# JaapWijnen/metal-raytracing

Measured on AMD Instinct MI355X. Metric: Mrays/sec (primary+shadow) and ms/frame, DragonScene 1920x1080 spp=1, higher is better.
Workload: dtype f32

## Files before the change

metal-raytracing_amd/csrc/api.cpp:

```cpp
#include "api_types.h"
#include "abi_check.h"
#include "../../include/mrt_debug.h"
#include <algorithm>
#include <cstring>
#include <cstdio>
#include <memory>
#include <new>

namespace mrt {
static thread_local std::string g_err;
void set_error(const std::string &msg) { g_err = msg; }
int hip_fail(hipError_t e, const char *what, const char *file, int line) {
    char buf[512];
    snprintf(buf, sizeof buf, "HIP error %d (%s) in %s at %s:%d", (int)e, hipGetErrorString(e), what, file, line);
    g_err = buf;
    return e == hipErrorOutOfMemory ? MRT_ERR_OUT_OF_MEMORY : MRT_ERR_HIP;
}
}

static int bind_device(MRTContext ctx) { MRT_HIP(hipSetDevice(ctx->device)); return MRT_OK; }

static int sync_host_meshes(MRTScene scene) {
    bool pending = false;
    int rc = mrt::download_stale_meshes(scene->meshes, scene->dev, &pending);
// ... 723 lines not shown
    else { mrt::set_error("mrt_renderer_get_option: unknown key " + k); return MRT_ERR_INVALID_ARGUMENT; }
    return MRT_OK;
    MRT_CATCH
}
int mrt_debug_renderer_set_option(MRTRenderer r, const char *key, double value) {
    MRT_TRY
    REQUIRE(r && key, "mrt_debug_renderer_set_option: bad argument");
    std::string k(key);
    if (k == "persistent") { REQUIRE(value == 0 || value == 1 || value == 2, "persistent must be 0 (never), 1 (always) or 2 (by launch size)"); r->r.persistent = (int)value; }
    else if (k == "xcd_counters") { REQUIRE(value == 0 || value == 1, "xcd_counters must be 0 or 1"); r->r.xcd_counters = (int)value; }
    else if (k == "tile_groups") { REQUIRE(value >= 0 && value <= mrt::MAX_TILE_GROUPS && value == (int)value, "tile_groups must be 0 (by the draw), 1 (never) or 2..4"); r->r.tile_groups = (int)value; }
    else if (k == "shade_pack") { REQUIRE(value == 0 || value == 1, "shade_pack must be 0 or 1"); r->r.shade_pack = (int)value; }
    else if (k == "hit_lds") { REQUIRE(value == 0 || value == 1, "hit_lds must be 0 or 1"); r->r.hit_lds = (int)value; }
    else if (k == "persist_chunk") { REQUIRE(value >= 64 && value <= 65536 && ((int)value % 64) == 0, "persist_chunk must be a multiple of 64 in [64, 65536]"); r->r.persist_chunk = (int)value; }
    else if (k == "wave_slots") { REQUIRE(value >= 1 && value <= (1 << 20), "wave_slots must be in [1, 2^20]"); r->r.wave_slots = (int)value; r->r.wave_slots_user = true; }
    else if (k == "stream_stride") { REQUIRE(value >= 0 && value <= 2, "stream_stride must be 0 (contiguous ranges), 1 (round-robin batches) or 2 (round-robin for a shard's launches)"); r->r.stream_stride = (int)value; }
    else if (k == "halton_table") r->r.halton_table = value != 0;
    else if (k == "equal_passes") r->r.equal_passes = value != 0;
    else if (k == "frame_bundle") { REQUIRE(value == 0 || value == 1, "frame_bundle must be 0 (off) or 1 (the sub-frames of a slot side by side in a wave)"); r->r.frame_bundle = (int)value; }
    else if (k == "stream_even") { REQUIRE(value >= 0 && value <= 1600, "stream_even must be in [0,1600] (percent of the wave slots; 0 = off)"); r->r.stream_even = (int)value; }
    else if (k == "primary_hint") r->r.primary_hint = value != 0;
    else if (k == "throughput_chain") r->r.throughput_chain = value != 0;
    else if (k == "shadow_planes") r->r.shadow_planes = value != 0 ? 1 : 0;
    else if (k == "tail_accumulate") r->r.tail_accumulate = value != 0;
    else if (k == "fuse_primary") { REQUIRE(value == 0 || value == 1 || value == 2, "fuse_primary must be 0, 1 (not for one frame alone) or 2 (always)"); r->r.fuse_primary = (int)value; }
    else if (k == "wide_bounce") r->r.wide_bounce = value != 0;
    else if (k == "tl_pair_cap") { REQUIRE(value >= 0 && value <= 4294967295.0, "tl_pair_cap out of range"); r->r.tl_pair_cap = (int)std::min(value, 2147483647.0); }
    else if (k == "tl_pairs") { REQUIRE(value == 0 || value == 1 || value == 2, "tl_pairs must be 0 (two-level scenes walked in one loop), 1 (TLAS pass + BLAS pass over (ray, instance) pairs) or 2 (the same, the TLAS pass always as a walk of the 8-wide TLAS)"); r->r.tl_pairs = (int)value; }
    else if (k == "primary_wide") { REQUIRE(value == 0 || value == 1 || value == 2, "primary_wide must be 0 (rope walk inside shade(0)), 1 (own launch of the 8-wide stream kernel) or 2 (8-wide walk inside shade(0))"); r->r.primary_wide = (int)value; }
    else return mrt_renderer_set_option(r, key, value);
    return MRT_OK;
    MRT_CATCH
}
int mrt_debug_renderer_get_option(MRTRenderer r, const char *key, double *value) {
    MRT_TRY
    REQUIRE(r && key && value, "mrt_debug_renderer_get_option: bad argument");
    std::string k(key);
    if (k == "persistent") *value = r->r.persistent;
    else if (k == "persist_chunk") *value = r->r.persist_chunk;
    else if (k == "hit_lds") *value = r->r.hit_lds;
    else if (k == "shade_pack") *value = r->r.shade_pack;
    else if (k == "tile_groups") *value = r->r.tile_groups;
    else if (k == "groups_used") *value = r->r.groups_used;
    else if (k == "xcd_counters") *value = r->r.xcd_counters;
    else if (k == "wave_slots") *value = r->r.wave_slots;
    else if (k == "stream_stride") *value = r->r.stream_stride;
    else if (k == "halton_table") *value = r->r.halton_table;
    else if (k == "frame_bundle") *value = r->r.frame_bundle;
    else if (k == "stream_even") *value = r->r.stream_even;
    else if (k == "primary_hint") *value = r->r.primary_hint ? 1 : 0;
    else if (k == "throughput_chain") *value = r->r.throughput_chain ? 1 : 0;
    else if (k == "shadow_planes") *value = r->r.shadow_planes;
    else if (k == "tail_accumulate") *value = r->r.tail_accumulate ? 1 : 0;
    else if (k == "fuse_primary") *value = r->r.fuse_primary;
    else if (k == "wide_bounce") *value = r->r.wide_bounce ? 1 : 0;
    else if (k == "tl_pairs") *value = r->r.tl_pairs;
    else if (k == "tl_pair_cap") *value = r->r.tl_pair_cap;
    else if (k == "primary_wide") *value = r->r.primary_wide;
    else return mrt_renderer_get_option(r, key, value);
    return MRT_OK;
    MRT_CATCH
}
int mrt_renderer_set_shard(MRTRenderer r, int32_t rank, int32_t world) {
    MRT_TRY
    RENDERER_PROLOGUE("mrt_renderer_set_shard")
    return r->r.set_shard(rank, world);
    MRT_CATCH
}
int mrt_renderer_set_frame_index(MRTRenderer r, uint32_t fi) { REQUIRE(r, "mrt_renderer_set_frame_index: NULL"); r->r.frame_index = fi; return MRT_OK; }
int mrt_renderer_frame_index(MRTRenderer r, uint32_t *fi) { REQUIRE(r && fi, "mrt_renderer_frame_index: bad argument"); *fi = r->r.frame_index; return MRT_OK; }
int mrt_renderer_render(MRTRenderer r, int32_t n_frames) {
    MRT_TRY
    RENDERER_PROLOGUE("mrt_renderer_render")
    REQUIRE(n_frames >= 0, "mrt_renderer_render: n_frames < 0");
    if (!r->scene->committed) { mrt::set_error("mrt_renderer_render: scene was modified and not re-committed"); return MRT_ERR_STATE; }
    if (n_frames == 0) return MRT_OK;
// ... 265 lines not shown
```

metal-raytracing_amd/csrc/renderer.h:

```cpp
#pragma once
#include "scene_device.h"
#include "host_geometry.h"
#include <algorithm>
#include <array>
#include <deque>
#include <vector>

namespace mrt {

struct EvPair { hipEvent_t a = nullptr, b = nullptr; int kind = 0; };

struct FrameLane {
    hipStream_t stream = nullptr;
    hipEvent_t accumulated = nullptr;
    DevBuf<float4> sample;
    DevBuf<float4> rayA[2], rayB[2], thr[2], hits, srayA, srayB, scon;
    DevBuf<unsigned long long> bounce_counts;
    DevBuf<float4> f_con[2];
    DevBuf<uint8_t> f_lit;
    DevBuf<uint4> pairs;
};
constexpr int MAX_FRAMES_IN_FLIGHT = 16;
constexpr int MAX_TILE_GROUPS = 4;
struct TileGroup { int rank = 0, world = 1, tiles_local = 0; uint32_t capacity = 0; uint64_t owned = 0; const uint32_t *seeds = nullptr; };
// ... 34 lines not shown
    uint32_t mega_waves = 0;
};
struct SlotCache { size_t lds_bytes = ~(size_t)0; int per_cu = 0; };
struct DrawCtx;

struct Renderer {
    hipStream_t stream = nullptr;
    const DeviceScene *scene = nullptr;
    int width = 0, height = 0, max_bounces = 3;
    uint32_t seed = 1;
    MRTCamera camera{};
    uint32_t frame_index = 0;
    uint32_t sample_offset = 0;
    int cur = 0;
    int shard_rank = 0, shard_world = 1;
    int tiles_local = 0;
    uint32_t capacity = 0;
    uint64_t owned_pixels = 0;
    uint64_t frames_rendered = 0;

    DevBuf<uint32_t> seeds;
    DevBuf<float> halton_tab;
    uint32_t halton_w0 = 0;
    int halton_table = 1;
    int ensure_halton_table(uint32_t sample_index, uint32_t frames);
    DevBuf<uint32_t> hint;
    bool primary_hint = true;
    bool throughput_chain = true;
    DevBuf<float4> accum[2];
    FrameLane lanes[MAX_FRAMES_IN_FLIGHT];
    int frames_in_flight = 3;
    int frame_batch = 0;
    int batch_wanted() const;
    int tile_groups = 0;
    int groups_used = 1;
    TileGroup tgroups[MAX_TILE_GROUPS];
    DevBuf<uint32_t> seeds_g[MAX_TILE_GROUPS]; int tgroups_for = 0, tgroups_batch = 0;
    int ensure_tile_groups(int G);
    int lanes_used = 0;
    int lanes_ready = 0;
    int alloc_batch = 0;
    bool megakernel = false;
    bool materials = false;
    int primary_wide = 2;
    int persistent = 2;
    int xcd_counters = 1;
    int hit_lds = 1;
    int shade_pack = 1;
    int persist_chunk = 256;
    int wave_slots = 7168;
    bool wave_slots_user = false;
    mutable SlotCache mega_cache, persist_cache, persist_x_cache;
    mutable int cu_count = 0;
    int alloc_planes(FrameLane &L);
    bool tail_accumulate = true;
    int fuse_primary = 1;
    int shadow_planes = 1;
    int equal_passes = 1;
    int frame_bundle = 1;
    int stream_stride = 2;
    int stream_even = 200;
    int tl_pair_cap = 0;
    int tl_pairs = 1;
    bool wide_bounce = true;
    hipEvent_t ev_fork = nullptr;
    DevBuf<unsigned long long> totals;

    bool guides = false;
    bool guides_valid = false;
    bool guides_keep = false;
    DevBuf<float4> guide_nd, guide_albedo; DevBuf<int4> guide_ids;
    hipStream_t guide_stream = nullptr;
    hipEvent_t guide_fork = nullptr, guide_done = nullptr;
    DevBuf<float4> dn_scratch[2], denoised; bool denoised_valid = false;
    int set_guides(bool on);
    int ensure_guides();
    int clear_guides();
    int read_guide(int which, void *out, size_t nbytes);
// ... 14 lines not shown
    hipEvent_t ev_begin = nullptr, ev_end = nullptr;
    std::array<EvPair, 512> ev_ext;
    int ext_used = 0;
    bool pending_timing = false;
    float ms_last = 0, ms_extend_last = 0; uint32_t extend_launches_last = 0;
    MRTKernelTimes kernel_times{};

    Renderer() = default;
    Renderer(const Renderer &) = delete;
    ~Renderer();
    int init(hipStream_t st, const DeviceScene *sc, int w, int h, uint32_t seed, int max_bounces);
    int resize(int w, int h);
    int alloc_queues();
    int alloc_lane(FrameLane &L);
    void release_lane(FrameLane &L);
    size_t lane_bytes() const;
    int set_shard(int rank, int world);
    int render(int n_frames);
    DrawPlan plan_draw(int n_frames) const;
    int plan_pass(const DrawPlan &dp, const SceneView &sv, const TileGroup &TG, int B, PassPlan &pp) const;
    PullGrid pull_grid(size_t slots, size_t slots_of_chip, size_t min_chunk, bool long_call) const;
    int draw_nothing(int n_frames);
    int rebuild_for_batch();
    int ensure_lanes(int want);
    void begin_draw(DrawCtx &d) const;
    int prepare_lane(FrameLane &L, const TileGroup &TG, const PassPlan &pp);
    int enqueue_pass(DrawCtx &d, FrameLane &L, const TileGroup &TG, const PassPlan &pp, int pass, int g);
    int enqueue_megakernel_pass(DrawCtx &d, FrameLane &L, const TileGroup &TG, const PassPlan &pp);
    void enqueue_primary(DrawCtx &d, FrameLane &L, const TileGroup &TG, const PassPlan &pp);
    void enqueue_shade(DrawCtx &d, FrameLane &L, const TileGroup &TG, const PassPlan &pp, int b);
    void enqueue_trace(DrawCtx &d, FrameLane &L, const TileGroup &TG, const PassPlan &pp, int b);
    int enqueue_accumulate(DrawCtx &d, FrameLane &L, const TileGroup &TG, const PassPlan &pp, int pass, int g);
    int enqueue_guides(DrawCtx &d);
    EvPair *timed(int kind);
    int wait();
    int read_accum(float *rgba, size_t nbytes);
    int copy_accum_to_device(void *dptr, size_t nbytes);
    int write_accum_from_device(const void *dptr, size_t nbytes);
    int read_tonemapped(uint8_t *rgba, size_t nbytes);
    int pack_owned_tiles(void *dptr, size_t nbytes);
    int unpack_tiles(const void *dptr, size_t nbytes, int rank, int world);
    int stats(MRTRenderStats *out);
    int reset_stats();
};

uint32_t shard_tiles(int width, int height, int rank, int world);
int unpack_tiles_into(float4 *image, int width, int height, const void *compact, size_t nbytes, int rank, int world, hipStream_t st);
// ... 15 lines not shown
```

metal-raytracing_amd/csrc/renderer.hip:

```cpp
#include <hip/hip_ext.h>
#include "renderer.h"
#include "device_math.h"
#include "traverse.h"
#include "traverse_wide.h"
#include "traverse_instanced.h"
#include "shade.h"
#include "two_level_passes.h"
#include <cstdlib>
#include <cstring>
#include <algorithm>

namespace mrt {
namespace {

__global__ void k_halton_table(float *__restrict__ tab, uint32_t w0, uint32_t n) {
    const uint32_t j = blockIdx.x * blockDim.x + threadIdx.x;
    if (j < n) tab[MRT_HALTON_INTERLEAVED ? (size_t)j * HALTON_TAB_DIMS + blockIdx.y : (size_t)blockIdx.y * n + j] = halton_dev((int)(w0 + j), (int)blockIdx.y + 1);
}

__global__ void k_seed(uint32_t *__restrict__ seeds, uint32_t n, uint32_t seed) {
    uint32_t i = blockIdx.x * blockDim.x + threadIdx.x;
    if (i < n) seeds[(size_t)blockIdx.y * n + i] = seed_hash_dev(seed, i) + blockIdx.y;
}

// ... 583 lines not shown

static inline uint32_t cdiv(size_t a, size_t b) { return (uint32_t)((a + b - 1) / b); }

template <class... KArgs, class... Args>
static inline void launch_timed(EvPair *ev, void (*kernel)(KArgs...), dim3 grid, dim3 block, size_t shmem, hipStream_t st, Args... args) {
    if (ev) hipExtLaunchKernelGGL(kernel, grid, block, (uint32_t)shmem, st, ev->a, ev->b, 0, static_cast<KArgs>(args)...);
    else hipLaunchKernelGGL(kernel, grid, block, shmem, st, static_cast<KArgs>(args)...);
}

}

#ifdef MRT_WAVE_TIMES
int read_wave_times(unsigned long long *out) { return hipMemcpyFromSymbol(out, HIP_SYMBOL(g_wave_times), sizeof(g_wave_times)) == hipSuccess ? MRT_OK : MRT_ERR_HIP; }
int read_wave_iters(uint32_t *out) { return hipMemcpyFromSymbol(out, HIP_SYMBOL(g_wave_iters), sizeof(g_wave_iters)) == hipSuccess ? MRT_OK : MRT_ERR_HIP; }
int read_drain_probe(unsigned long long *out18, int reset) {
    if (hipMemcpyFromSymbol(out18, HIP_SYMBOL(g_drain_probe), sizeof(g_drain_probe)) != hipSuccess) return MRT_ERR_HIP;
    if (reset) { static const unsigned long long z[18] = {0}; if (hipMemcpyToSymbol(HIP_SYMBOL(g_drain_probe), z, sizeof z) != hipSuccess) return MRT_ERR_HIP; }
    return MRT_OK;
}
#endif

int Renderer::ensure_halton_table(uint32_t sample_index, uint32_t frames) {
    const uint64_t first_pass = std::min<uint64_t>(frames, MAX_FRAME_BATCH);
    const bool fits = halton_tab.p != nullptr && sample_index >= halton_w0 && (uint64_t)sample_index + first_pass + (1u << 20) <= (uint64_t)halton_w0 + HALTON_TAB_SPAN;
    if (fits) return MRT_OK;
    if (!halton_tab.p) MRT_HIP(halton_tab.alloc((size_t)HALTON_TAB_DIMS * HALTON_TAB_SPAN));
    halton_w0 = sample_index;
    hipLaunchKernelGGL(k_halton_table, dim3(cdiv(HALTON_TAB_SPAN, 256), HALTON_TAB_DIMS), dim3(256), 0, stream, halton_tab.p, halton_w0, HALTON_TAB_SPAN);
    MRT_HIP(hipGetLastError());
    return MRT_OK;
}

int Renderer::init(hipStream_t st, const DeviceScene *sc, int w, int h, uint32_t seed_, int max_bounces_) {
    stream = st; scene = sc; seed = seed_; max_bounces = max_bounces_;
    MRT_HIP(hipEventCreate(&ev_begin)); MRT_HIP(hipEventCreate(&ev_end));
    MRT_HIP(hipEventCreateWithFlags(&ev_fork, hipEventDisableTiming));
    for (auto &e : ev_ext) { MRT_HIP(hipEventCreate(&e.a)); MRT_HIP(hipEventCreate(&e.b)); }
    for (auto &L : lanes) {
        MRT_HIP(hipStreamCreateWithFlags(&L.stream, hipStreamNonBlocking));
        MRT_HIP(hipEventCreateWithFlags(&L.accumulated, hipEventDisableTiming));
        MRT_HIP(L.bounce_counts.alloc(WORK_COUNTERS + 32 * WORK_COUNTERS_PER_BOUNCE));
        MRT_HIP(hipMemsetAsync(L.bounce_counts.p, 0, L.bounce_counts.bytes(), stream));
    }
    MRT_HIP(totals.alloc(4));
    MRT_HIP(hipMemsetAsync(totals.p, 0, totals.bytes(), stream));
    return resize(w, h);
}

Renderer::~Renderer() {
    if (ev_begin) (void)hipEventDestroy(ev_begin);
    if (ev_end) (void)hipEventDestroy(ev_end);
    if (ev_fork) (void)hipEventDestroy(ev_fork);
    for (auto &e : ev_ext) { if (e.a) (void)hipEventDestroy(e.a); if (e.b) (void)hipEventDestroy(e.b); }
    for (auto &pd : passes_pending) (void)hipEventDestroy(pd.ev);
    for (auto e : pass_events_free) (void)hipEventDestroy(e);
    if (guide_stream) { (void)hipStreamSynchronize(guide_stream); (void)hipStreamDestroy(guide_stream); }
    if (guide_done) (void)hipEventDestroy(guide_done);
    if (guide_fork) (void)hipEventDestroy(guide_fork);
    for (auto &L : lanes) {
        if (L.stream) { (void)hipStreamSynchronize(L.stream); (void)hipStreamDestroy(L.stream); }
        if (L.accumulated) (void)hipEventDestroy(L.accumulated);
    }
}

int Renderer::batch_wanted() const {
    if (frame_batch > 0) return std::min(frame_batch, MAX_FRAME_BATCH);
    const size_t owned = std::max<size_t>(1, (size_t)std::max(width, 1) * (size_t)std::max(height, 1) / (size_t)std::max(shard_world, 1));
    const size_t ref = (size_t)DEFAULT_FRAME_BATCH * 1920 * 1080;
// ... 101 lines not shown
    for (int k = 0; k < 2; k++) { MRT_HIP(L.rayA[k].alloc(qcap)); MRT_HIP(L.rayB[k].alloc(qcap)); if (need_thr) MRT_HIP(L.thr[k].alloc(qcap)); }
    MRT_HIP(L.hits.alloc(qcap)); MRT_HIP(L.srayA.alloc(qcap)); MRT_HIP(L.srayB.alloc(qcap));
    if (need_thr || !shadow_planes) MRT_HIP(L.scon.alloc(qcap));
    MRT_HIP(L.sample.alloc((size_t)std::max<uint32_t>(capacity, 1u) * (size_t)std::max(1, alloc_batch)));
    MRT_HIP(hipMemsetAsync(L.sample.p, 0, L.sample.bytes(), stream));
    if (shadow_planes && !need_thr) { if (int rc = alloc_planes(L)) return rc; }
    return MRT_OK;
}

int Renderer::ensure_tile_groups(int G) {
    const int Bq = std::max(1, alloc_batch);
    if (tgroups_for == G && tgroups_batch == Bq) return MRT_OK;
    const int tiles_x = (width + 7) / 8, tiles_y = (height + 7) / 8, tiles = tiles_x * tiles_y;
    for (int g = 0; g < G; g++) {
        TileGroup &T = tgroups[g];
        T.rank = g * shard_world + shard_rank; T.world = G * shard_world;
        T.tiles_local = std::max(0, (tiles - T.rank + T.world - 1) / T.world);
        T.capacity = (uint32_t)T.tiles_local * 64u;
        T.owned = 0;
        for (int lt = 0; lt < T.tiles_local; lt++) {
            const int tile = lt * T.world + T.rank, ty = tile / tiles_x, tx = tile % tiles_x;
            T.owned += (uint64_t)std::min(8, width - tx * 8) * (uint64_t)std::min(8, height - ty * 8);
        }
        MRT_HIP(seeds_g[g].alloc((size_t)std::max<uint32_t>(T.capacity, 1u) * Bq));
        FrameParams sp{}; sp.width = width; sp.height = height; sp.shard_rank = T.rank; sp.shard_world = T.world; sp.tiles_x = tiles_x; sp.tiles_local = T.tiles_local; sp.capacity = T.capacity;
        if (T.capacity) hipLaunchKernelGGL(k_seed_slots, dim3(cdiv(T.capacity, 256), Bq), dim3(256), 0, stream, seeds_g[g].p, sp, seed);
        T.seeds = seeds_g[g].p;
    }
    tgroups_for = G; tgroups_batch = Bq;
    return MRT_OK;
}

int Renderer::set_shard(int rank, int world) {
    if (world < 1 || rank < 0 || rank >= world) { set_error("invalid shard"); return MRT_ERR_INVALID_ARGUMENT; }
    shard_rank = rank; shard_world = world;
    MRT_HIP(hipStreamSynchronize(stream));
    MRT_HIP(hipMemsetAsync(accum[0].p, 0, accum[0].bytes(), stream));
    MRT_HIP(hipMemsetAsync(accum[1].p, 0, accum[1].bytes(), stream));
    frame_index = 0; cur = 0;
    if (int rc = clear_guides()) return rc;
    return alloc_queues();
}

int Renderer::clear_guides() {
    guides_valid = false; denoised_valid = false;
    if (guide_nd.p) {
        MRT_HIP(hipMemsetAsync(guide_nd.p, 0, guide_nd.bytes(), stream)); MRT_HIP(hipMemsetAsync(guide_albedo.p, 0, guide_albedo.bytes(), stream));
        MRT_HIP(hipMemsetAsync(guide_ids.p, 0, guide_ids.bytes(), stream));
    }
    return MRT_OK;
}
int Renderer::set_guides(bool on) {
// ... 67 lines not shown
    int rc = wait(); if (rc) return rc;
    MRT_HIP(hipMemcpy(rgba, tmp.p, nbytes, hipMemcpyDeviceToHost));
    return MRT_OK;
}

#ifdef MRT_DIAGNOSTICS
static inline int ablate_mask() { static const int mask = getenv("MRT_ABLATE") ? atoi(getenv("MRT_ABLATE")) : 0; return mask; }
#else
static constexpr int ablate_mask() { return 0; }
#endif
static inline uint32_t tag_bounce(uint32_t arg, int b) {
#ifdef MRT_WAVE_TIMES
    return arg | ((uint32_t)b << 24);
#else
    (void)b; return arg;
#endif
}

struct DrawCtx {
    SceneView sv;
    DrawPlan dp;
    FrameParams fp;
    FrameParams gp;
    hipEvent_t last_acc, last_acc_g[MAX_TILE_GROUPS];
    AccGroup tail;
};

template <class K>
static int wave_slots_for(K kernel, size_t lds_bytes, SlotCache &cache, int &cu_count) {
    if (cu_count == 0) { int dev = 0; hipDeviceProp_t prop; MRT_HIP(hipGetDevice(&dev)); MRT_HIP(hipGetDeviceProperties(&prop, dev)); cu_count = prop.multiProcessorCount; }
    if (cache.lds_bytes != lds_bytes) { MRT_HIP(hipOccupancyMaxActiveBlocksPerMultiprocessor(&cache.per_cu, kernel, 64, lds_bytes)); cache.lds_bytes = lds_bytes; }
    return MRT_OK;
}

EvPair *Renderer::timed(int kind) { if (ext_used >= (int)ev_ext.size()) return nullptr; ev_ext[ext_used].kind = kind; return &ev_ext[ext_used++]; }

DrawPlan Renderer::plan_draw(int n_frames) const {
    DrawPlan dp;
    dp.n_frames = n_frames; dp.mega = megakernel; dp.equal = equal_passes != 0; dp.tail = tail_accumulate;
    const int batch_cap = alloc_batch > DEFAULT_FRAME_BATCH ? std::min(alloc_batch, std::max(DEFAULT_FRAME_BATCH, (n_frames + 2) / 3)) : alloc_batch;
    dp.batch_max = megakernel ? 1 : batch_cap;
    dp.n_passes = (n_frames + dp.batch_max - 1) / dp.batch_max;
    dp.lanes = dp.lanes_plain = std::max(1, std::min(frames_in_flight, MAX_FRAMES_IN_FLIGHT));
    if (!megakernel && tile_groups != 1 && tiles_local >= 64) {
        const int in_flight = std::max(1, std::min(dp.lanes, dp.n_passes));
        const int by_draw = tile_groups >= 2 ? tile_groups : dp.batch_max > 1 ? 1 : in_flight == 1 ? 3 : in_flight <= 3 ? 2 : 1;
        dp.G = std::max(1, std::min(by_draw, std::min(MAX_FRAMES_IN_FLIGHT / in_flight, tiles_local / 32)));
        if (dp.G > 1) dp.lanes = in_flight * dp.G;
    }
    return dp;
}

void DrawPlan::settle(int lanes_ready) {
    if (G > 1 && lanes_ready < lanes) { G = 1; lanes = lanes_plain; }
    lanes = std::min(lanes, lanes_ready);
    Fp = G > 1 ? lanes / G : lanes;
    tail_from = (tail && G == 1) ? n_passes - std::min(lanes, n_passes) : n_passes;
    long_call = n_passes >= 2 * lanes;
}

PullGrid Renderer::pull_grid(size_t slots, size_t slots_of_chip, size_t min_chunk, bool long_call) const {
    PullGrid pg;
    pg.chunk = (uint32_t)std::min<size_t>((size_t)persist_chunk, std::max<size_t>(min_chunk, slots / (slots_of_chip * 4) / 64 * 64));
    pg.grid_slots = (!wave_slots_user && long_call) ? std::max<size_t>(1, slots_of_chip / 2) : slots_of_chip;
    pg.waves = (uint32_t)std::max<size_t>(1, std::min<size_t>(cdiv(slots, pg.chunk), pg.grid_slots));
    return pg;
// ... 74 lines not shown
    return MRT_OK;
}

int Renderer::rebuild_for_batch() {
    MRT_HIP(hipStreamSynchronize(stream));
    const uint32_t keep_frame = frame_index; const int keep_cur = cur; const uint64_t keep_rendered = frames_rendered;
    DevBuf<float4> keep; MRT_HIP(keep.alloc(accum[cur].n));
    MRT_HIP(hipMemcpyAsync(keep.p, accum[cur].p, accum[cur].bytes(), hipMemcpyDeviceToDevice, stream));
    const MRTCamera keep_cam = camera;
    unsigned long long keep_totals[3] = {0, 0, 0};
    MRT_HIP(hipMemcpy(keep_totals, totals.p, sizeof keep_totals, hipMemcpyDeviceToHost));
    const bool keep_denoised = denoised_valid;
    guides_keep = true;
    int rc = resize(width, height);
    guides_keep = false; denoised_valid = keep_denoised;
    if (rc) return rc;
    MRT_HIP(hipMemcpyAsync(totals.p, keep_totals, sizeof keep_totals, hipMemcpyHostToDevice, stream));
    MRT_HIP(hipMemcpyAsync(accum[keep_cur].p, keep.p, keep.bytes(), hipMemcpyDeviceToDevice, stream));
    MRT_HIP(hipStreamSynchronize(stream));
    frame_index = keep_frame; cur = keep_cur; frames_rendered = keep_rendered; frames_completed_known = keep_rendered; camera = keep_cam;
    return MRT_OK;
}

int Renderer::ensure_lanes(int want) {
    for (; lanes_ready < want; lanes_ready++) {
        const size_t need = lane_bytes() + (lanes_ready == 0 && !halton_tab.p ? (size_t)HALTON_TAB_DIMS * HALTON_TAB_SPAN * sizeof(float) : 0);
        size_t free_b = 0, total_b = 0;
        const bool fits = hipMemGetInfo(&free_b, &total_b) != hipSuccess || free_b > need + (size_t(1) << 30);
        int rc = fits ? alloc_lane(lanes[lanes_ready]) : MRT_ERR_OUT_OF_MEMORY;
        if (rc == MRT_ERR_OUT_OF_MEMORY && lanes_ready >= 1) { (void)hipGetLastError(); release_lane(lanes[lanes_ready]); break; }
        if (rc == MRT_ERR_OUT_OF_MEMORY) { set_error("not enough device memory for one pass in flight: " + std::to_string(need >> 20) + " MiB of ray queues needed (" + std::to_string(width) + "x" + std::to_string(height) + ", frame_batch " + std::to_string(alloc_batch) + "); lower frame_batch"); return rc; }
        if (rc) return rc;
    }
    return MRT_OK;
}

void Renderer::begin_draw(DrawCtx &d) const {
    FrameParams &fp = d.fp;
    fp = FrameParams{};
    fp.width = width; fp.height = height; fp.lightCount = light_count_limit > 0 ? std::min(light_count_limit, d.sv.light_count) : d.sv.light_count;
    fp.cam_pos = make_float4(camera.position.x, camera.position.y, camera.position.z, 0);
    fp.cam_right = make_float4(camera.right.x, camera.right.y, camera.right.z, 0);
    fp.cam_up = make_float4(camera.up.x, camera.up.y, camera.up.z, 0);
    fp.cam_fwd = make_float4(camera.forward.x, camera.forward.y, camera.forward.z, 0);
    fp.shard_rank = shard_rank; fp.shard_world = shard_world;
    fp.tiles_x = (width + 7) / 8; fp.tiles_local = tiles_local; fp.max_bounces = max_bounces;
    d.gp = fp;
    d.gp.frameIndex = frame_index; d.gp.sampleIndex = frame_index + sample_offset; d.gp.npix = (uint32_t)((size_t)width * height); d.gp.capacity = capacity; d.gp.batch = 1;
    fp.npix = (uint32_t)((size_t)width * height); fp.capacity = capacity;
    d.last_acc = nullptr;
    for (hipEvent_t &e : d.last_acc_g) e = nullptr;
    d.tail.n = 0;
}

int Renderer::prepare_lane(FrameLane &L, const TileGroup &TG, const PassPlan &pp) {
    const size_t shard_qcap = (size_t)capacity * (size_t)std::max(1, alloc_batch);
    if (!pp.chain && !L.thr[0].p) {
        for (int k = 0; k < 2; k++) MRT_HIP(L.thr[k].alloc(shard_qcap));
    }
    if (pp.planes) {
        if (!L.f_lit.p) { if (int rc = alloc_planes(L)) return rc; }
        MRT_HIP(hipMemsetAsync(L.f_lit.p, 0, 4 * (size_t)TG.capacity * (size_t)pp.B, L.stream));
    }
    if (pp.pairs && !L.pairs.p) MRT_HIP(L.pairs.alloc(std::max<size_t>(PairQueue::WORDS * pp.pair_cap, 1)));
    if (!pp.planes && !L.scon.p) MRT_HIP(L.scon.alloc(shard_qcap));
    return MRT_OK;
}

int Renderer::enqueue_megakernel_pass(DrawCtx &d, FrameLane &L, const TileGroup &TG, const PassPlan &pp) {
    FrameParams &fp = d.fp;
    uint32_t *work = reinterpret_cast<uint32_t *>(L.bounce_counts.p + 64);
    for (int sub = 0; sub < pp.B; sub++) {
        fp.frameIndex = frame_index + (uint32_t)sub; fp.sampleIndex = frame_index + (uint32_t)sub + sample_offset; fp.batch = 1;
        if (d.last_acc) { MRT_HIP(hipStreamWaitEvent(L.stream, d.last_acc, 0)); d.last_acc = nullptr; }
        MRT_HIP(hipMemsetAsync(work, 0, 4, L.stream));
        launch_timed(timed(MRT_KERNEL_TRACE), k_megakernel, dim3(pp.mega_waves), dim3(64), pp.stack_bytes, L.stream, d.sv, fp, TG.seeds, accum[cur].p, accum[1 - cur].p, work, totals.p, (uint32_t)TG.owned);
        cur = 1 - cur;
    }
    MRT_HIP(hipEventRecord(L.accumulated, L.stream));
    d.last_acc = L.accumulated;
    frame_index += (uint32_t)pp.B; frames_rendered += (uint64_t)pp.B;
    return note_pass(L.stream);
}

void Renderer::enqueue_primary(DrawCtx &d, FrameLane &L, const TileGroup &TG, const PassPlan &pp) {
    if (pp.primary == PrimaryForm::none) return;
    float4 *const dirs = L.rayB[1].p;
    uint32_t *const hint_p = pp.primary_hinted ? hint.p : nullptr;
    if (pp.primary == PrimaryForm::stream) {
        const auto kernel = pp.two_level ? (pp.primary_hinted ? k_trace_primary_wide_stream<true, true> : k_trace_primary_wide_stream<true, false>)
                                         : (pp.primary_hinted ? k_trace_primary_wide_stream<false, true> : k_trace_primary_wide_stream<false, false>);
        launch_timed(timed(MRT_KERNEL_PRIMARY), kernel, dim3(cdiv(TG.capacity, pp.rpw_p), pp.B), dim3(64), pp.stack_bytes, L.stream, d.sv, d.fp, TG.seeds, L.hits.p, dirs, TG.capacity, pp.rpw_p, hint_p);
        return;
    }
    const bool lane_wide = pp.primary == PrimaryForm::lane_wide;
    auto kernel = k_trace_primary<true>;
    if (!pp.two_level) kernel = lane_wide ? k_trace_primary<false, true> : k_trace_primary<false>;
    launch_timed(timed(MRT_KERNEL_PRIMARY), kernel, dim3(pp.grid_tiles, pp.B), dim3(64), lane_wide ? pp.stack_bytes : 0, L.stream, d.sv, d.fp, TG.seeds, L.hits.p, dirs, hint_p);
}

using ShadeKernel = void (*)(SceneView, FrameParams, const uint32_t *, const float4 *, const float4 *, const float4 *, const float4 *, const unsigned long long *, uint32_t, float4 *, float4 *, float4 *, float4 *, float4 *, float4 *,
                             unsigned long long *, float4 *, float4 *, uint32_t *);
static ShadeKernel shade_kernel_for(const PassPlan &pp, bool materials, bool pack, int b) {
    if (pack) return materials ? (ShadeKernel)k_shade_pack<true, false, false, false>
                   : pp.pairs ? (ShadeKernel)k_shade_pack<false, true, true, true>
                   : pp.planes ? (ShadeKernel)k_shade_pack<false, true, true, false>
                   : pp.chain ? (ShadeKernel)k_shade_pack<false, true, false, false> : (ShadeKernel)k_shade_pack<false, false, false, false>;
    return materials ? (ShadeKernel)k_shade<true, false, false, false>
         : (pp.pairs && b > 0) ? (ShadeKernel)k_shade<false, true, true, true>
         : (pp.trace0_wide && b == 0 && pp.two_level) ? (ShadeKernel)k_shade_primary<3>
         : (pp.trace0_wide && b == 0) ? (ShadeKernel)k_shade_primary<2>
// ... 3 lines not shown
}

void Renderer::enqueue_shade(DrawCtx &d, FrameLane &L, const TileGroup &TG, const PassPlan &pp, int b) {
    FrameParams &fp = d.fp;
    const int q = b & 1, B = pp.B;
    unsigned long long *const bc = L.bounce_counts.p;
    fp.bounce = b;
    const bool pack = shade_pack && b > 0;
    fp.pack_range = pp.pack_range;
    fp.frame_bundle = (pp.bundle && b == 0) ? 1 : 0;
    if (fp.frame_bundle) {
        fp.bundle_groups = ((uint32_t)B + 7u) / 8u; fp.bundle_w = ((uint32_t)B + fp.bundle_groups - 1u) / fp.bundle_groups;
        fp.bundle_per_wave = 64u / fp.bundle_w; fp.bundle_magic = (65536u + fp.bundle_w - 1u) / fp.bundle_w;
    }
    fp.halton_tab = nullptr; fp.halton_w0 = 0; fp.halton_n = 0;
    if (fp.frame_bundle && fp.bundle_w >= 4u && halton_table && halton_tab.p) {
        fp.halton_tab = halton_tab.p; fp.halton_w0 = halton_w0; fp.halton_n = HALTON_TAB_SPAN;
    }
    const dim3 gs = b == 0 ? (fp.frame_bundle ? dim3(cdiv(cdiv((size_t)TG.capacity * fp.bundle_groups, fp.bundle_per_wave) * 64, SHADE_THREADS), 1) : dim3(pp.grid_shade, B)) : dim3(cdiv((size_t)TG.capacity * B, pack ? fp.pack_range : (uint32_t)SHADE_THREADS));
    float4 *const con_b = !pp.planes ? L.scon.p : b == 0 ? L.sample.p : L.f_con[b - 1].p;
    const size_t shade_lds = (pp.trace0_wide && b == 0) ? (size_t)SHADE_WAVES * (scene->wide_depth * WIDE_STACK_LEVEL_BYTES + (MRT_LANE_HIT_LDS ? 1024 : 0)) : 0;
    launch_timed(timed(MRT_KERNEL_SHADE), shade_kernel_for(pp, materials, pack, b), gs, dim3(SHADE_THREADS), shade_lds, L.stream, d.sv, fp, TG.seeds, L.rayA[1 - q].p, L.rayB[1 - q].p, L.thr[1 - q].p, L.hits.p,
                 b == 0 ? nullptr : bc + (b - 1), TG.capacity, L.rayA[q].p, L.rayB[q].p, L.thr[q].p, L.srayA.p, L.srayB.p, con_b, bc + b, b == 0 ? L.sample.p : nullptr, L.sample.p,
                 (b == 0 && pp.trace0_pass && pp.trace0_hint) ? hint.p : nullptr);
}

void Renderer::enqueue_trace(DrawCtx &d, FrameLane &L, const TileGroup &TG, const PassPlan &pp, int b) {
    if (ablate_mask() & 2) return;
    const int q = b & 1;
    hipStream_t st = L.stream;
    unsigned long long *const bc = L.bounce_counts.p;
    const unsigned long long *const counts = bc + b;
    uint32_t *const work = reinterpret_cast<uint32_t *>(bc + WORK_COUNTERS + (size_t)b * WORK_COUNTERS_PER_BOUNCE);
    uint8_t *const lit_b = pp.planes ? L.f_lit.p + b : nullptr;
    const float4 *const rayA = L.rayA[q].p, *const rayB = L.rayB[q].p, *const srayA = L.srayA.p, *const srayB = L.srayB.p;
    const uint32_t xcd_frames = xcd_counters ? (uint32_t)pp.B : 0u;
    switch (pp.trace) {
    case TraceForm::pairs: {
        unsigned long long *const keys = reinterpret_cast<unsigned long long *>(L.hits.p);
        uint32_t *const pc = reinterpret_cast<uint32_t *>(bc + 65 + b);
        const uint32_t stack_words = (uint32_t)(pp.stack_bytes / 4);
        if (pp.tl_flat) launch_timed(timed(MRT_KERNEL_TRACE), k_tl_top_flat, dim3((uint32_t)std::max<size_t>(1, std::min<size_t>(cdiv(2 * (size_t)TG.capacity * pp.B, 64), 2 * pp.pg.grid_slots))), dim3(64), pp.stack_bytes + 8, st, d.sv, rayA, rayB, keys, srayA, srayB,
                                     counts, lit_b, L.pairs.p, pc, pp.pair_cap_used, stack_words);
        else launch_timed(timed(MRT_KERNEL_TRACE), k_tl_top, dim3(pp.pg.waves), dim3(64), pp.stack_bytes + 8, st, d.sv, rayA, rayB, keys, srayA, srayB,
                          counts, reinterpret_cast<uint32_t *>(bc + 32 + b), pp.pg.chunk, lit_b, L.pairs.p, pc, pp.pair_cap_used, stack_words);
        launch_timed(timed(MRT_KERNEL_TRACE), k_tl_blas, dim3((uint32_t)pp.pg.grid_slots), dim3(64), (size_t)scene->wide_depth * WIDE_STACK_LEVEL_BYTES, st, d.sv, rayA, rayB, keys, srayA, srayB,
                     counts, pc + 1, 256u, lit_b, (const uint4 *)L.pairs.p, (const uint32_t *)pc, pp.pair_cap_used);
// ... 61 lines not shown

int Renderer::enqueue_guides(DrawCtx &d) {
    const bool two_level = d.sv.num_inst > 0;
    const size_t lds = d.sv.num_wnodes ? (size_t)scene->wide_depth * WIDE_STACK_LEVEL_BYTES : 0;
    const auto kernel = two_level ? (d.sv.num_wnodes ? k_guides<3> : k_guides<0>) : (d.sv.num_wnodes ? k_guides<2> : k_guides<1>);
    hipLaunchKernelGGL(kernel, dim3(std::max<uint32_t>(1u, (uint32_t)tiles_local)), dim3(64), lds, guide_stream, d.sv, d.gp, (const uint32_t *)seeds.p, (uint32_t)d.dp.n_frames, guide_nd.p, guide_albedo.p, guide_ids.p);
    const hipError_t le = hipGetLastError();
    (void)hipEventRecord(guide_done, guide_stream);
    (void)hipStreamWaitEvent(stream, guide_done, 0);
    if (le != hipSuccess) return hip_fail(le, "k_guides launch", __FILE__, __LINE__);
    guides_valid = true;
    return MRT_OK;
}

int Renderer::render(int n_frames) {
    if (!scene) { set_error("renderer has no scene"); return MRT_ERR_STATE; }
    DrawCtx d;
    d.sv = scene->view();
    if (d.sv.light_count < 1) { set_error("scene has no lights (lightCount must be >= 1, Raytracing.metal:273)"); return MRT_ERR_STATE; }
    if (tiles_local == 0) return draw_nothing(n_frames);
    if (alloc_batch != batch_wanted()) { if (int rc = rebuild_for_batch()) return rc; return render(n_frames); }
    DrawPlan &dp = d.dp;
    dp = plan_draw(n_frames);
    if (int rc = ensure_lanes(dp.lanes)) return rc;
    dp.settle(lanes_ready);
    lanes_used = dp.lanes; groups_used = dp.G;
    if (dp.G > 1) { if (int rc = ensure_tile_groups(dp.G)) return rc; }
    const TileGroup self_group{shard_rank, shard_world, tiles_local, capacity, owned_pixels, seeds.p};
    PassPlan plans[2][MAX_TILE_GROUPS];
    for (int k = 0; k < 2; k++)
        for (int g = 0; g < dp.G; g++) { if (int rc = plan_pass(dp, d.sv, dp.G > 1 ? tgroups[g] : self_group, dp.pass_size(k == 0 ? 0 : dp.n_passes - 1), plans[k][g])) return rc; }
    wave_slots = plans[0][0].wave_slots;
    begin_draw(d);
    ext_used = 0;
    if (halton_table && frame_bundle && !megakernel && n_frames > 1) { if (int rc = ensure_halton_table(frame_index + sample_offset, (uint32_t)n_frames)) return rc; }
    MRT_HIP(hipEventRecord(ev_begin, stream));
    MRT_HIP(hipEventRecord(ev_fork, stream));
    for (int k = 0; k < dp.lanes; k++) MRT_HIP(hipStreamWaitEvent(lanes[k].stream, ev_fork, 0));
    if (guides) {
        if (int rc = ensure_guides()) return rc;
        MRT_HIP(hipEventRecord(guide_fork, stream));
        MRT_HIP(hipStreamWaitEvent(guide_stream, guide_fork, 0));
    }
    for (int pass = 0; pass < dp.n_passes; pass++) {
        const int B = dp.pass_size(pass);
        for (int g = 0; g < dp.G; g++) {
            const TileGroup &TG = dp.G > 1 ? tgroups[g] : self_group;
            if (dp.G > 1 && TG.capacity == 0) continue;
// ... 246 lines not shown
```

Measured before the change: 14390.

## Prime new frame lanes with a tiny warm-up draw and preallocate per-lane buffers

When new frame lanes are created, their plan-dependent buffers, the tile-group seed buffers, the Halton table and a pool of pass events are allocated up front. Each new lane then runs a one-tile warm-up pass through primary, shade, trace and accumulate into scratch memory, and its counters are reset afterwards. The aim is to move first-use allocation and kernel-loading costs out of the measured draws. This costs extra memory and setup work, and the warm-up must leave no state behind, for example through the shared hint buffer, which is why it uses a separate scratch hint.

```diff
diff --git a/metal-raytracing_amd/csrc/api.cpp b/metal-raytracing_amd/csrc/api.cpp
--- a/metal-raytracing_amd/csrc/api.cpp
+++ b/metal-raytracing_amd/csrc/api.cpp
@@ -769,7 +769,8 @@
     else if (k == "primary_hint") r->r.primary_hint = value != 0;
     else if (k == "throughput_chain") r->r.throughput_chain = value != 0;
     else if (k == "shadow_planes") r->r.shadow_planes = value != 0 ? 1 : 0;
-    else if (k == "tail_accumulate") r->r.tail_accumulate = value != 0;
+    else if (k == "tail_accumulate") { REQUIRE(value == 0 || value == 1 || value == 2, "tail_accumulate must be 0 (every pass accumulates on its lane), 1 (the draw's last passes in one launch after the join) or 2 (by the draw)"); r->r.tail_accumulate = (int)value; }
+    else if (k == "prime_lanes") { REQUIRE(value == 0 || value == 1, "prime_lanes must be 0 or 1"); r->r.prime_lanes = (int)value; }
     else if (k == "fuse_primary") { REQUIRE(value == 0 || value == 1 || value == 2, "fuse_primary must be 0, 1 (not for one frame alone) or 2 (always)"); r->r.fuse_primary = (int)value; }
     else if (k == "wide_bounce") r->r.wide_bounce = value != 0;
     else if (k == "tl_pair_cap") { REQUIRE(value >= 0 && value <= 4294967295.0, "tl_pair_cap out of range"); r->r.tl_pair_cap = (int)std::min(value, 2147483647.0); }
@@ -798,7 +799,8 @@
     else if (k == "primary_hint") *value = r->r.primary_hint ? 1 : 0;
     else if (k == "throughput_chain") *value = r->r.throughput_chain ? 1 : 0;
     else if (k == "shadow_planes") *value = r->r.shadow_planes;
-    else if (k == "tail_accumulate") *value = r->r.tail_accumulate ? 1 : 0;
+    else if (k == "tail_accumulate") *value = r->r.tail_accumulate;
+    else if (k == "prime_lanes") *value = r->r.prime_lanes;
     else if (k == "fuse_primary") *value = r->r.fuse_primary;
     else if (k == "wide_bounce") *value = r->r.wide_bounce ? 1 : 0;
     else if (k == "tl_pairs") *value = r->r.tl_pairs;
diff --git a/metal-raytracing_amd/csrc/renderer.h b/metal-raytracing_amd/csrc/renderer.h
--- a/metal-raytracing_amd/csrc/renderer.h
+++ b/metal-raytracing_amd/csrc/renderer.h
@@ -80,6 +80,7 @@
     DevBuf<uint32_t> seeds;
     DevBuf<float> halton_tab;
     uint32_t halton_w0 = 0;
+    bool halton_filled = false;
     int halton_table = 1;
     int ensure_halton_table(uint32_t sample_index, uint32_t frames);
     DevBuf<uint32_t> hint;
@@ -95,6 +96,7 @@
     TileGroup tgroups[MAX_TILE_GROUPS];
     DevBuf<uint32_t> seeds_g[MAX_TILE_GROUPS]; int tgroups_for = 0, tgroups_batch = 0;
     int ensure_tile_groups(int G);
+    int reserve_tile_groups();
     int lanes_used = 0;
     int lanes_ready = 0;
     int alloc_batch = 0;
@@ -111,7 +113,9 @@
     mutable SlotCache mega_cache, persist_cache, persist_x_cache;
     mutable int cu_count = 0;
     int alloc_planes(FrameLane &L);
-    bool tail_accumulate = true;
+    int tail_accumulate = 2;
+    int prime_lanes = 1;
+    DevBuf<float4> prime_scratch;
     int fuse_primary = 1;
     int shadow_planes = 1;
     int equal_passes = 1;
@@ -172,7 +176,9 @@
     PullGrid pull_grid(size_t slots, size_t slots_of_chip, size_t min_chunk, bool long_call) const;
     int draw_nothing(int n_frames);
     int rebuild_for_batch();
-    int ensure_lanes(int want);
+    int ensure_lanes(DrawPlan &dp, const SceneView &sv);
+    int alloc_for_plan(FrameLane &L, const PassPlan &pp);
+    int prime_lane(FrameLane &L, const DrawPlan &dp, const SceneView &sv, const PassPlan &full);
     void begin_draw(DrawCtx &d) const;
     int prepare_lane(FrameLane &L, const TileGroup &TG, const PassPlan &pp);
     int enqueue_pass(DrawCtx &d, FrameLane &L, const TileGroup &TG, const PassPlan &pp, int pass, int g);
diff --git a/metal-raytracing_amd/csrc/renderer.hip b/metal-raytracing_amd/csrc/renderer.hip
--- a/metal-raytracing_amd/csrc/renderer.hip
+++ b/metal-raytracing_amd/csrc/renderer.hip
@@ -629,15 +629,16 @@
 
 int Renderer::ensure_halton_table(uint32_t sample_index, uint32_t frames) {
     const uint64_t first_pass = std::min<uint64_t>(frames, MAX_FRAME_BATCH);
-    const bool fits = halton_tab.p != nullptr && sample_index >= halton_w0 && (uint64_t)sample_index + first_pass + (1u << 20) <= (uint64_t)halton_w0 + HALTON_TAB_SPAN;
+    const bool fits = halton_filled && sample_index >= halton_w0 && (uint64_t)sample_index + first_pass + (1u << 20) <= (uint64_t)halton_w0 + HALTON_TAB_SPAN;
     if (fits) return MRT_OK;
     if (!halton_tab.p) MRT_HIP(halton_tab.alloc((size_t)HALTON_TAB_DIMS * HALTON_TAB_SPAN));
-    halton_w0 = sample_index;
+    halton_w0 = sample_index; halton_filled = true;
     hipLaunchKernelGGL(k_halton_table, dim3(cdiv(HALTON_TAB_SPAN, 256), HALTON_TAB_DIMS), dim3(256), 0, stream, halton_tab.p, halton_w0, HALTON_TAB_SPAN);
     MRT_HIP(hipGetLastError());
     return MRT_OK;
 }
 
+constexpr size_t PRIME_TOTALS_AT = 128, PRIME_HINT_AT = 130;
 int Renderer::init(hipStream_t st, const DeviceScene *sc, int w, int h, uint32_t seed_, int max_bounces_) {
     stream = st; scene = sc; seed = seed_; max_bounces = max_bounces_;
     MRT_HIP(hipEventCreate(&ev_begin)); MRT_HIP(hipEventCreate(&ev_end));
@@ -651,6 +652,10 @@
     }
     MRT_HIP(totals.alloc(4));
     MRT_HIP(hipMemsetAsync(totals.p, 0, totals.bytes(), stream));
+    for (int k = 0; k < MAX_FRAMES_IN_FLIGHT * 4; k++) { hipEvent_t e = nullptr; MRT_HIP(hipEventCreateWithFlags(&e, hipEventDisableTiming)); pass_events_free.push_back(e); }
+    MRT_HIP(prime_scratch.alloc(PRIME_HINT_AT + 16));
+    MRT_HIP(hipMemsetAsync(prime_scratch.p, 0, prime_scratch.bytes(), stream));
+    MRT_HIP(hipMemsetAsync(prime_scratch.p + PRIME_HINT_AT, 0xFF, 64 * sizeof(uint32_t), stream));
     return resize(w, h);
 }
 
@@ -798,12 +803,25 @@
             const int tile = lt * T.world + T.rank, ty = tile / tiles_x, tx = tile % tiles_x;
             T.owned += (uint64_t)std::min(8, width - tx * 8) * (uint64_t)std::min(8, height - ty * 8);
         }
-        MRT_HIP(seeds_g[g].alloc((size_t)std::max<uint32_t>(T.capacity, 1u) * Bq));
+        if (seeds_g[g].n < (size_t)std::max<uint32_t>(T.capacity, 1u) * Bq) MRT_HIP(seeds_g[g].alloc((size_t)std::max<uint32_t>(T.capacity, 1u) * Bq));
         FrameParams sp{}; sp.width = width; sp.height = height; sp.shard_rank = T.rank; sp.shard_world = T.world; sp.tiles_x = tiles_x; sp.tiles_local = T.tiles_local; sp.capacity = T.capacity;
         if (T.capacity) hipLaunchKernelGGL(k_seed_slots, dim3(cdiv(T.capacity, 256), Bq), dim3(256), 0, stream, seeds_g[g].p, sp, seed);
         T.seeds = seeds_g[g].p;
     }
     tgroups_for = G; tgroups_batch = Bq;
+    return MRT_OK;
+}
+
+int Renderer::reserve_tile_groups() {
+    const int reach = (megakernel || tile_groups == 1 || tiles_local < 64) ? 1 : tile_groups >= 2 ? tile_groups : alloc_batch == 1 ? 3 : 1;
+    const int Gmax = std::min(reach, std::min(MAX_TILE_GROUPS, tiles_local / 32));
+    const int tiles = ((width + 7) / 8) * ((height + 7) / 8);
+    for (int g = 0; g < Gmax && Gmax > 1; g++) {
+        int most = 0;
+        for (int G = std::max(2, g + 1); G <= Gmax; G++) most = std::max(most, (tiles - (g * shard_world + shard_rank) + G * shard_world - 1) / (G * shard_world));
+        const size_t need = (size_t)std::max(most * 64, 1) * (size_t)std::max(1, alloc_batch);
+        if (seeds_g[g].n < need) { MRT_HIP(seeds_g[g].alloc(need)); tgroups_for = 0; }
+    }
     return MRT_OK;
 }
 
@@ -917,6 +935,7 @@
     DrawPlan dp;
     FrameParams fp;
     FrameParams gp;
+    uint32_t *hint;
     hipEvent_t last_acc, last_acc_g[MAX_TILE_GROUPS];
     AccGroup tail;
 };
@@ -932,11 +951,12 @@
 
 DrawPlan Renderer::plan_draw(int n_frames) const {
     DrawPlan dp;
-    dp.n_frames = n_frames; dp.mega = megakernel; dp.equal = equal_passes != 0; dp.tail = tail_accumulate;
+    dp.n_frames = n_frames; dp.mega = megakernel; dp.equal = equal_passes != 0;
     const int batch_cap = alloc_batch > DEFAULT_FRAME_BATCH ? std::min(alloc_batch, std::max(DEFAULT_FRAME_BATCH, (n_frames + 2) / 3)) : alloc_batch;
     dp.batch_max = megakernel ? 1 : batch_cap;
     dp.n_passes = (n_frames + dp.batch_max - 1) / dp.batch_max;
     dp.lanes = dp.lanes_plain = std::max(1, std::min(frames_in_flight, MAX_FRAMES_IN_FLIGHT));
+    dp.tail = tail_accumulate != 0;
     if (!megakernel && tile_groups != 1 && tiles_local >= 64) {
         const int in_flight = std::max(1, std::min(dp.lanes, dp.n_passes));
         const int by_draw = tile_groups >= 2 ? tile_groups : dp.batch_max > 1 ? 1 : in_flight == 1 ? 3 : in_flight <= 3 ? 2 : 1;
@@ -1057,8 +1077,9 @@
     return MRT_OK;
 }
 
-int Renderer::ensure_lanes(int want) {
-    for (; lanes_ready < want; lanes_ready++) {
+int Renderer::ensure_lanes(DrawPlan &dp, const SceneView &sv) {
+    const int first_new = lanes_ready;
+    for (; lanes_ready < dp.lanes; lanes_ready++) {
         const size_t need = lane_bytes() + (lanes_ready == 0 && !halton_tab.p ? (size_t)HALTON_TAB_DIMS * HALTON_TAB_SPAN * sizeof(float) : 0);
         size_t free_b = 0, total_b = 0;
         const bool fits = hipMemGetInfo(&free_b, &total_b) != hipSuccess || free_b > need + (size_t(1) << 30);
@@ -1067,6 +1088,64 @@
         if (rc == MRT_ERR_OUT_OF_MEMORY) { set_error("not enough device memory for one pass in flight: " + std::to_string(need >> 20) + " MiB of ray queues needed (" + std::to_string(width) + "x" + std::to_string(height) + ", frame_batch " + std::to_string(alloc_batch) + "); lower frame_batch"); return rc; }
         if (rc) return rc;
     }
+    dp.settle(lanes_ready);
+    if (lanes_ready == first_new) return MRT_OK;
+    if (first_new == 0) {
+        if (halton_table && frame_bundle && !megakernel && alloc_batch > 1 && !halton_tab.p) MRT_HIP(halton_tab.alloc((size_t)HALTON_TAB_DIMS * HALTON_TAB_SPAN));
+        if (int rc = reserve_tile_groups()) return rc;
+    }
+    const int tl_g = (tiles_local + dp.G - 1) / dp.G;
+    const TileGroup first_group{shard_rank, shard_world, tl_g, (uint32_t)tl_g * 64u, 0, seeds.p};
+    PassPlan pp;
+    if (int rc = plan_pass(dp, sv, first_group, dp.pass_size(0), pp)) return rc;
+    for (int k = first_new; k < lanes_ready; k++) {
+        if (!dp.mega) { if (int rc = alloc_for_plan(lanes[k], pp)) return rc; }
+        if (prime_lanes) { if (int rc = prime_lane(lanes[k], dp, sv, pp)) return rc; }
+    }
+    return MRT_OK;
+}
+
+int Renderer::prime_lane(FrameLane &L, const DrawPlan &dp, const SceneView &sv, const PassPlan &full) {
+    const TileGroup tile{0, 1, 1, 64u, 64, seeds.p};
+    PassPlan pp = full;
+    pp.B = 1; pp.grid_tiles = 1; pp.grid_shade = 1; pp.bundle = false; pp.pack_range = 2 * SHADE_THREADS;
+    pp.pg.waves = 1; pp.pg.grid_slots = 1; pp.mega_waves = 1;
+    if (pp.even) pp.even = std::min<uint32_t>(pp.even, 2u);
+    pp.static_grid = pp.even ? pp.even : cdiv(2 * 64, std::max<uint32_t>(pp.rpw_m, 64u));
+    DrawCtx d;
+    d.sv = sv; d.dp = dp;
+    begin_draw(d);
+    FrameParams &fp = d.fp;
+    fp.width = 8; fp.height = 8; fp.npix = 64; fp.tiles_x = 1;
+    fp.shard_rank = tile.rank; fp.shard_world = tile.world; fp.tiles_local = tile.tiles_local; fp.capacity = tile.capacity;
+    fp.batch = 1; fp.frameIndex = frame_index; fp.sampleIndex = frame_index + sample_offset;
+    d.hint = reinterpret_cast<uint32_t *>(prime_scratch.p + PRIME_HINT_AT);
+    float4 *const prev = prime_scratch.p, *const dst = prime_scratch.p + 64;
+    unsigned long long *const tot = reinterpret_cast<unsigned long long *>(prime_scratch.p + PRIME_TOTALS_AT);
+    unsigned long long *const bc = L.bounce_counts.p;
+    hipStream_t st = L.stream;
+    ext_used = 0;
+    MRT_HIP(hipEventRecord(ev_fork, stream));
+    MRT_HIP(hipStreamWaitEvent(st, ev_fork, 0));
+    if (dp.mega) {
+        uint32_t *work = reinterpret_cast<uint32_t *>(bc + 64);
+        MRT_HIP(hipMemsetAsync(work, 0, 4, st));
+        launch_timed(timed(MRT_KERNEL_TRACE), k_megakernel, dim3(1), dim3(64), pp.stack_bytes, st, d.sv, fp, tile.seeds, (const float4 *)prev, dst, work, tot, 64u);
+    } else {
+        if (int rc = prepare_lane(L, tile, pp)) return rc;
+        fp.bounce = 0; fp.chain = pp.chain ? 1 : 0;
+        fp.wide_stack_words = (uint32_t)((size_t)scene->wide_depth * WIDE_STACK_LEVEL_BYTES / 4);
+        enqueue_primary(d, L, tile, pp);
+        for (int b = 0; b < max_bounces; b++) { enqueue_shade(d, L, tile, pp, b); enqueue_trace(d, L, tile, pp, b); }
+        if (pp.planes) launch_timed(timed(MRT_KERNEL_ACCUMULATE), k_accumulate_planes, dim3(1), dim3(64), 0, st, fp, L.sample.p, L.f_con[0].p, L.f_con[1].p, L.f_lit.p, prev, dst, bc, tot, 64u);
+        else launch_timed(timed(MRT_KERNEL_ACCUMULATE), k_accumulate, dim3(1), dim3(64), 0, st, fp, L.sample.p, prev, dst, bc, tot, 64u);
+    }
+    MRT_HIP(hipGetLastError());
+    MRT_HIP(hipMemsetAsync(bc, 0, L.bounce_counts.bytes(), st));
+    MRT_HIP(hipMemsetAsync(L.sample.p, 0, 64 * sizeof(float4), st));
+    MRT_HIP(hipEventRecord(L.accumulated, st));
+    MRT_HIP(hipStreamWaitEvent(stream, L.accumulated, 0));
+    ext_used = 0;
     return MRT_OK;
 }
 
@@ -1083,22 +1162,25 @@
     d.gp = fp;
     d.gp.frameIndex = frame_index; d.gp.sampleIndex = frame_index + sample_offset; d.gp.npix = (uint32_t)((size_t)width * height); d.gp.capacity = capacity; d.gp.batch = 1;
     fp.npix = (uint32_t)((size_t)width * height); fp.capacity = capacity;
+    d.hint = hint.p;
     d.last_acc = nullptr;
     for (hipEvent_t &e : d.last_acc_g) e = nullptr;
     d.tail.n = 0;
 }
 
-int Renderer::prepare_lane(FrameLane &L, const TileGroup &TG, const PassPlan &pp) {
+int Renderer::alloc_for_plan(FrameLane &L, const PassPlan &pp) {
     const size_t shard_qcap = (size_t)capacity * (size_t)std::max(1, alloc_batch);
     if (!pp.chain && !L.thr[0].p) {
         for (int k = 0; k < 2; k++) MRT_HIP(L.thr[k].alloc(shard_qcap));
     }
-    if (pp.planes) {
-        if (!L.f_lit.p) { if (int rc = alloc_planes(L)) return rc; }
-        MRT_HIP(hipMemsetAsync(L.f_lit.p, 0, 4 * (size_t)TG.capacity * (size_t)pp.B, L.stream));
-    }
+    if (pp.planes && !L.f_lit.p) { if (int rc = alloc_planes(L)) return rc; }
     if (pp.pairs && !L.pairs.p) MRT_HIP(L.pairs.alloc(std::max<size_t>(PairQueue::WORDS * pp.pair_cap, 1)));
     if (!pp.planes && !L.scon.p) MRT_HIP(L.scon.alloc(shard_qcap));
+    return MRT_OK;
+}
+int Renderer::prepare_lane(FrameLane &L, const TileGroup &TG, const PassPlan &pp) {
+    if (int rc = alloc_for_plan(L, pp)) return rc;
+    if (pp.planes) MRT_HIP(hipMemsetAsync(L.f_lit.p, 0, 4 * (size_t)TG.capacity * (size_t)pp.B, L.stream));
     return MRT_OK;
 }
 
@@ -1121,7 +1203,7 @@
 void Renderer::enqueue_primary(DrawCtx &d, FrameLane &L, const TileGroup &TG, const PassPlan &pp) {
     if (pp.primary == PrimaryForm::none) return;
     float4 *const dirs = L.rayB[1].p;
-    uint32_t *const hint_p = pp.primary_hinted ? hint.p : nullptr;
+    uint32_t *const hint_p = pp.primary_hinted ? d.hint : nullptr;
     if (pp.primary == PrimaryForm::stream) {
         const auto kernel = pp.two_level ? (pp.primary_hinted ? k_trace_primary_wide_stream<true, true> : k_trace_primary_wide_stream<true, false>)
                                          : (pp.primary_hinted ? k_trace_primary_wide_stream<false, true> : k_trace_primary_wide_stream<false, false>);
@@ -1171,7 +1253,7 @@
     const size_t shade_lds = (pp.trace0_wide && b == 0) ? (size_t)SHADE_WAVES * (scene->wide_depth * WIDE_STACK_LEVEL_BYTES + (MRT_LANE_HIT_LDS ? 1024 : 0)) : 0;
     launch_timed(timed(MRT_KERNEL_SHADE), shade_kernel_for(pp, materials, pack, b), gs, dim3(SHADE_THREADS), shade_lds, L.stream, d.sv, fp, TG.seeds, L.rayA[1 - q].p, L.rayB[1 - q].p, L.thr[1 - q].p, L.hits.p,
                  b == 0 ? nullptr : bc + (b - 1), TG.capacity, L.rayA[q].p, L.rayB[q].p, L.thr[q].p, L.srayA.p, L.srayB.p, con_b, bc + b, b == 0 ? L.sample.p : nullptr, L.sample.p,
-                 (b == 0 && pp.trace0_pass && pp.trace0_hint) ? hint.p : nullptr);
+                 (b == 0 && pp.trace0_pass && pp.trace0_hint) ? d.hint : nullptr);
 }
 
 void Renderer::enqueue_trace(DrawCtx &d, FrameLane &L, const TileGroup &TG, const PassPlan &pp, int b) {
@@ -1279,8 +1361,7 @@
     if (alloc_batch != batch_wanted()) { if (int rc = rebuild_for_batch()) return rc; return render(n_frames); }
     DrawPlan &dp = d.dp;
     dp = plan_draw(n_frames);
-    if (int rc = ensure_lanes(dp.lanes)) return rc;
-    dp.settle(lanes_ready);
+    if (int rc = ensure_lanes(dp, d.sv)) return rc;
     lanes_used = dp.lanes; groups_used = dp.G;
     if (dp.G > 1) { if (int rc = ensure_tile_groups(dp.G)) return rc; }
     const TileGroup self_group{shard_rank, shard_world, tiles_local, capacity, owned_pixels, seeds.p};
```

After: 14340. No clear change (-0.3%).
